# QData/FastSK

Measured on AMD Instinct MI355X. Metric: gkm kernel build: mismatch-combos/s, higher is better.
Workload: dtype u4 count planes (v_dot8_u32_u4), u32 register sums, u64 triangle (plain stores on the first pass over reset rows, else atomics); 1 GPU; config5: synthetic DNA 100000 x 300 bp, g=12 m=8 exact, 495 combos; n_seq=100000, seq_len=300, g=12, m=8, combos=495, parallelism=single GPU

## Files before the change

### fastsk_amd/csrc/fsk_engine_dense_shift.hip

```cpp
#include "fsk_engine_internal.h"
#include "fsk_kernels_dense_shift.h"

#include <map>

using namespace fsk_detail;

namespace fsk {

#define FSK_DMA_SHIFT 1
#define FSK_DMA_KERNEL k_dense_tile_shift
#define FSK_DMA_COMPACT 0
#include "fsk_tile_kernel_dma.inc"
#undef FSK_DMA_KERNEL
#undef FSK_DMA_SHIFT

#define FSK_DMA_SHIFT 2
#define FSK_DMA_KERNEL k_dense_tile_shift_all
#include "fsk_tile_kernel_dma.inc"
#undef FSK_DMA_KERNEL
#undef FSK_DMA_COMPACT
#undef FSK_DMA_SHIFT

}

// ... 101 lines not shown
int dense_shift_edge_keys(fsk_engine* e, const uint8_t* chunk_pos, uint32_t panels_pad) {
    ShiftPlan& p = e->shift;
    const uint32_t n_steps = (uint32_t)(p.steps.size() / 2), np_seq = panels_pad * fsk::PANEL;
    std::vector<uint32_t> steps = p.steps;
    dense_shift_unpack_flags(steps, p.n_bases, e->tune.dense_shift_batch != 0);
    const std::vector<uint32_t> chain_tab = dense_shift_chain_table(steps, p.n_bases);
    FSK_HIP(e->d_shift_steps.reserve(p.steps.size() + p.group_steps.size() + chain_tab.size()));
    FSK_HIP(e->d_edge_keys.reserve((size_t)n_steps * np_seq));
    FSK_HIP(hipMemcpyAsync(e->d_shift_steps.p, steps.data(), steps.size() * sizeof(uint32_t), hipMemcpyHostToDevice, e->stream));
    if (!p.group_steps.empty())
        FSK_HIP(hipMemcpyAsync(e->d_shift_steps.p + p.steps.size(), p.group_steps.data(), p.group_steps.size() * sizeof(uint32_t), hipMemcpyHostToDevice,
                               e->stream));
    if (!chain_tab.empty())
        FSK_HIP(hipMemcpyAsync(e->d_shift_steps.p + p.steps.size() + p.group_steps.size(), chain_tab.data(), chain_tab.size() * sizeof(uint32_t),
                               hipMemcpyHostToDevice, e->stream));
    e->ld.shift_chains = (uint32_t)(chain_tab.size() / 2);
    FSK_LAUNCH(fsk::k_dense_edge_keys, dim3(panels_pad, (n_steps + 3u) / 4u), dim3(256), 0, e->stream, e->view(), e->cfg.g, e->k, e->sigma, chunk_pos,
               (const uint32_t*)e->d_shift_steps.p, n_steps, np_seq, e->d_edge_keys.p);
    FSK_HIP(hipStreamSynchronize(e->stream));
    e->st.launches += 1;
    return FSK_OK;
}

int dense_shift_keymajor(fsk_engine* e, uint32_t panels_pad, int nb, uint32_t Vq8) {
    const ShiftPlan& p = e->shift;
    e->ld.shift_packed = false;
    if (e->tune.dense_shift_packed < 0 || p.max_chain != SHIFT_PACKED_CHAIN) return FSK_OK;
    const size_t plane = (size_t)panels_pad * Vq8 * fsk::PANEL * (size_t)nb;
    const size_t n_keys = (p.steps.size() / 2) * (size_t)panels_pad * fsk::PANEL;
    const size_t want = (2 * plane + n_keys) * sizeof(uint32_t);
    const char* why = nullptr;
    if (e->tune.dense_shift_plane_kb > 0 && want > (size_t)e->tune.dense_shift_plane_kb * 1024) why = "over the dense_shift_plane_kb cap";
    const size_t grow = (std::max(plane, e->d_KM.cap) - e->d_KM.cap + std::max(plane, e->d_KMH.cap) - e->d_KMH.cap +
                         std::max(n_keys, e->d_edge_offs.cap) - e->d_edge_offs.cap) * sizeof(uint32_t);
    if (!why && grow > 0) {
        size_t free_b = 0, total_b = 0;
        if (hipMemGetInfo(&free_b, &total_b) != hipSuccess) free_b = 0;
        if (grow > free_b / 2) why = "more than half of the free device memory";
        else if (e->d_KM.reserve(plane) != hipSuccess || e->d_KMH.reserve(plane) != hipSuccess || e->d_edge_offs.reserve(n_keys) != hipSuccess) {
            (void)hipGetLastError();
            e->d_KM.release(); e->d_KMH.release(); e->d_edge_offs.release();
            why = "hipMalloc failed";
        }
    }
    if (why) {
        if (e->trace())
            fprintf(stderr, "[fsk] dense shift classes: the key-major planes (%.1f MB) do not fit, %s: k_dense_shift_fix runs the corrections\n",
                    (double)want / 1e6, why);
        return FSK_OK;
    }
    const uint32_t n_pairs = panels_pad / 2u;
    const uint32_t kgrid = (uint32_t)(((size_t)n_pairs * nb * Vq8 * 16u + 255u) / 256u);
    FSK_LAUNCH(fsk::k_dense_keymajor, dim3(kgrid), dim3(256), 0, e->stream, (const uint32_t*)e->d_C4.p, n_pairs, nb, Vq8, e->d_KM.p);
    FSK_LAUNCH(fsk::k_dense_keymajor, dim3(kgrid), dim3(256), 0, e->stream, (const uint32_t*)e->d_C4H.p, n_pairs, nb, Vq8, e->d_KMH.p);
    FSK_LAUNCH(fsk::k_dense_edge_offs, dim3((uint32_t)((n_keys + 255u) / 256u)), dim3(256), 0, e->stream, (const uint16_t*)e->d_edge_keys.p, n_keys,
               e->d_edge_offs.p);
    e->st.launches += 3;
    e->ld.shift_packed = true;
    return FSK_OK;
}

int dense_shift_tiles(fsk_engine* e, u64 n_tiles, int nb, uint32_t Vq8, uint32_t nst, u64* K, int store, uint32_t panels_pad) {
    const ShiftPlan& p = e->shift;
    const bool one_launch = !p.group_steps.empty() && (e->tune.dense_shift_one_launch > 0 ||
                                                       (e->tune.dense_shift_one_launch == 0 && e->tune.tile_splits == 0 && n_tiles >= 16384));
    int base_launches = 1;
    if (one_launch) {
        FSK_LAUNCH(fsk::k_dense_tile_shift_all, dim3((uint32_t)n_tiles, 1), dim3(256), 0, e->stream, (const uint32_t*)e->d_C4.p,
                   (const uint32_t*)e->d_C4H.p, (const uint32_t*)e->d_rowmask.p, (const uint32_t*)e->d_tiletab.p, nb, Vq8, nst, (uint32_t)e->N, K,
                   (int)p.n_bases, store, (const uint32_t*)e->d_shift_steps.p + p.steps.size());
    } else {
        base_launches = (int)(p.groups.size() / 2);
        int slot0 = 0;
        for (size_t gi = 0; gi + 1 < p.groups.size(); gi += 2) {
            const int end = (int)p.groups[gi];
            FSK_LAUNCH(fsk::k_dense_tile_shift, dim3((uint32_t)n_tiles, 1), dim3(256), 0, e->stream, (const uint32_t*)e->d_C4.p,
                       (const uint32_t*)e->d_C4H.p, (const uint32_t*)e->d_rowmask.p, (const uint32_t*)e->d_tiletab.p, nb, Vq8, nst, (uint32_t)e->N, K,
                       end - slot0, gi == 0 ? store : 0, slot0, p.groups[gi + 1]);
            slot0 = end;
        }
    }
    if (e->ld.shift_packed) {
        const bool ahead = e->tune.dense_shift_inplace != 0 && e->tune.dense_shift_ahead != 0 && e->ld.shift_chains > 0;
        const auto k_packed = ahead ? fsk::k_dense_shift_packed<true, true>
                                    : e->tune.dense_shift_inplace != 0 ? fsk::k_dense_shift_packed<true, false> : fsk::k_dense_shift_packed<false, false>;
        FSK_LAUNCH(k_packed, dim3((uint32_t)n_tiles), dim3(256), 0, e->stream, (const uint32_t*)e->d_KM.p, (const uint32_t*)e->d_KMH.p,
                   (const uint32_t*)e->d_rowmask.p, (const uint32_t*)e->d_tiletab.p,
                   (const uint32_t*)e->d_shift_steps.p + (ahead ? p.steps.size() + p.group_steps.size() : 0), (uint32_t)(p.steps.size() / 2),
                   (const uint32_t*)e->d_edge_offs.p, panels_pad * fsk::PANEL, nb, Vq8, ahead ? e->ld.shift_chains : p.n_bases, (uint32_t)(30u * p.wsum), (uint32_t)e->N, K);
    } else {
        FSK_LAUNCH(fsk::k_dense_shift_fix, dim3((uint32_t)n_tiles), dim3(512), 0, e->stream, (const uint32_t*)e->d_C4.p, (const uint32_t*)e->d_C4H.p,
                   (const uint32_t*)e->d_rowmask.p, (const uint32_t*)e->d_tiletab.p, (const uint32_t*)e->d_shift_steps.p, (uint32_t)(p.steps.size() / 2),
                   (const uint16_t*)e->d_edge_keys.p, panels_pad * fsk::PANEL, nb, Vq8, (uint32_t)e->N, K);
    }
    e->st.launches += (int32_t)base_launches;
    return FSK_OK;
}

}
```

### fastsk_amd/csrc/fsk_engine_internal.h

```cpp
#pragma once
#include "fsk_common.h"

#include <algorithm>
#include <chrono>
#include <cmath>
#include <cstdarg>
#include <cstdio>
#include <cstdlib>
#include <cstring>
#include <string>
#include <array>
#include <atomic>
#include <thread>
#include <vector>

#include <cstdint>
#include <climits>

#include "../../include/fastsk_amd.h"
#include <condition_variable>
#include <functional>
#include <memory>
#include <mutex>

// ... 21 lines not shown
        hipError_t r = hipMalloc((void**)&p, n * sizeof(T));
        if (r == hipSuccess) cap = n;
        return r;
    }
    void release() {
        if (p) (void)hipFree(p);
        p = nullptr;
        cap = 0;
    }
};

template <typename T>
struct PinnedBuf {
    T* p = nullptr;
    size_t cap = 0;
    PinnedBuf() = default;
    PinnedBuf(PinnedBuf&& o) noexcept : p(o.p), cap(o.cap) { o.p = nullptr; o.cap = 0; }
    PinnedBuf& operator=(PinnedBuf&& o) noexcept { std::swap(p, o.p); std::swap(cap, o.cap); return *this; }
    ~PinnedBuf() { release(); }
    hipError_t reserve(size_t n, size_t slack = 0) {
        if (n <= cap) return hipSuccess;
        release();
        hipError_t r = hipHostMalloc((void**)&p, (n + slack) * sizeof(T));
        if (r == hipSuccess) cap = n + slack;
        return r;
    }
    void release() {
        if (p) (void)hipHostFree(p);
        p = nullptr;
        cap = 0;
    }
};

template <typename H, hipError_t (*Create)(H*, unsigned), hipError_t (*Destroy)(H)>
struct Handle {
    H h = nullptr;
    Handle() = default;
    Handle(Handle&& o) noexcept : h(o.h) { o.h = nullptr; }
    Handle& operator=(Handle&& o) noexcept { std::swap(h, o.h); return *this; }
    ~Handle() { if (h) (void)Destroy(h); }
    hipError_t create(unsigned flags) { return h ? hipSuccess : Create(&h, flags); }
    operator H() const { return h; }
};
using Stream = Handle<hipStream_t, hipStreamCreateWithFlags, hipStreamDestroy>;
using Event = Handle<hipEvent_t, hipEventCreateWithFlags, hipEventDestroy>;

struct DeviceScope {
    int prev = -1, dev;
    hipError_t err = hipSuccess;
    explicit DeviceScope(int d) : dev(d) {
        if (hipGetDevice(&prev) != hipSuccess) prev = -1;
        if (prev != dev) err = hipSetDevice(dev);
    }
    ~DeviceScope() {
        if (prev >= 0 && prev != dev) (void)hipSetDevice(prev);
    }
    DeviceScope(const DeviceScope&) = delete;
    DeviceScope& operator=(const DeviceScope&) = delete;
};
#define FSK_ON_DEVICE(e)                                                                      \
    DeviceScope fsk_on_device_((e)->cfg.device);                                             \
    if (fsk_on_device_.err != hipSuccess)                                                    \
        return (e)->fail(FSK_EDEVICE, "hipSetDevice(%d) failed: %s", (e)->cfg.device, hipGetErrorString(fsk_on_device_.err))

}

using fsk_detail::DevBuf;
using fsk_detail::PinnedBuf;
using fsk_detail::Stream;
using fsk_detail::Event;

#define FSK_TUNING_KEYS(X)                                                                                                          \
    X(trace, 0, 0, 1, "stderr: the tuning in force, where the host time of a load and of a variance-mode call goes")                 \
    X(profile, -1, -1, 2, "fsk_config.profile from here on (-1: as the engine was created)")                                          \
    X(compact, -1, -1, 1, "dense: key compaction off / on whatever the alphabet says (-1: a rare symbol decides)")                   \
    X(compact_rare, -1, -1, 1, "dense: keys that occur from the places of the rare symbols (1) or a marking pass over every window (0)") \
    X(tile_splits, 0, 0, 4096, "dense: combo splits per tile (0: by the size of the launch)")                                        \
    X(dense_small, 0, 0, 1, "dense: 1 = a split tile launch (small N) leaves its sums as 32-bit staging blocks that k_dense_widen adds into K (0: one 64-bit atomic a cell and split — measured faster: the atomics drain under other workgroups' dot products)")                                        \
    X(dense_shift, 0, -1, 1, "dense: one weighted Gram product per chain of shifted combinations, the other members by edge lookups (fsk_engine_dense_shift.hip) — 1 = whenever the call is eligible, -1 = never (0: when eligible, tile_splits = 0 and the launch has 16384 tiles or more, the size from which a tile has one workgroup anyway)") \
    X(dense_shift_packed, 0, -1, 0, "dense, shift classes: the derived steps from key-major planes, eight cells an LDS read (k_dense_keymajor, k_dense_shift_packed; chains cut at nine members) — 0 = whenever the shift path runs and the planes fit, -1 = never: k_dense_shift_fix on the count panels") \
    X(dense_shift_inplace, 1, 0, 1, "dense, shift classes: k_dense_shift_packed stages a chain's first planes and makes every further step's in LDS, one nibble up and one down a sequence (a step that meets a count above 15 in its tile, and the step behind it, are staged) — 0 = every step staged") \
    X(dense_shift_batch, 1, 0, 1, "dense, shift classes: k_dense_shift_packed adds the prefix sums of several steps byte to byte and hands the bytes to its int32 sums once a batch, where the step table says so (a step at chain position r counts 30 (r + 1) against a byte's 255; a batch may span chains) — 0 = after every step") \
    X(dense_shift_ahead, 1, 0, 1, "dense, shift classes: k_dense_shift_packed stages the NEXT chain's first planes and key offsets at a chain's first step, into the idle stage buffer and an offsets ring in LDS (80 KB a workgroup), and issues no vector memory load inside a chain (a chain that meets a count above 15 in its tile stages as before) — 0 = every chain start staged one step ahead; ignored with dense_shift_inplace = 0 and on the k_dense_shift_fix path") \
    X(dense_shift_one_launch, 0, -1, 1, "dense, shift classes: every chain-length group of the base products in ONE launch that flushes at the group ends without clearing (k_dense_tile_shift_all) — 1 = whenever the shift path runs, -1 = never: one k_dense_tile_shift launch a group (0: where the shift path runs by its own default rule, tile_splits = 0 and 16384 tiles or more)") \
    X(dense_shift_plane_kb, 0, 0, (int64_t)1 << 40, "dense, shift classes: the key-major planes and offsets may take this many KiB at most (0: half of the free memory; tests: the planes do not fit)") \
    X(dense_chunk, 0, 0, 1 << 24, "dense: cap of the count kernel's staging chunk, in windows (0: none)")                             \
    X(variance_dense_slots, 1, 0, 1, "variance mode, dense: 0 = zero fill + k_welford per iteration instead of storing slot triangles") \
    X(var_slots16, 1, 0, 1, "variance mode, sparse: 0 = u32 slot triangles from the start")                                          \
    X(sparse_global, 0, 0, 1, "sparse: every += as a 64-bit atomicAdd (k_sx_emit<DIRECT>) whatever N is")                             \
    X(sparse_unpacked, 0, 0, 1, "sparse: entries in the general 8 + 4 (+ 4) byte format whatever N is")                               \
    X(sparse_pairs, 1, 0, 1, "sparse: 0 = every update word 32 bits wide (1: unit products of clean runs travel two to a word)")      \
    X(sparse_sync, 0, 0, 1, "sparse: wait for every batch's word count and size its stream exactly")                                 \
    X(sparse_hint, 1, 0, 1, "sparse: 0 = the words per record of the previous set of sequences are never kept as a hint")             \
    X(sparse_exact_lanes, 0, 0, 2, "sparse: the batches of an exact accumulate never (1) / always (2) in two lanes (0: from six batches on)") \
    X(sparse_batch_records, 0, 0, (int64_t)1 << 31, "sparse: records per batch at most (0: 2^27)")                                   \
    X(guard_cap, 0, 0, (int64_t)1 << 40, "sparse: pretend the stream buffer holds this many words (0: its real size)")                \
    X(list_max_words, 0, 0, (int64_t)1 << 31, "sparse: update words of one batch beyond which its pairs go to K with atomics (0: 2^31)") \
    X(seg_scan_chunked, 0, 0, 1, "sparse: the three-launch segment scan whatever the tile count")                                    \
    X(extract_slots, 0, 0, 4, "sparse: slots per k_sx_extract_win workgroup, 1 or 4 (0: by the size of the launch)")                  \
    X(sparse_form, 0, 0, 3, "sparse: the update stage — 1 = owner bands whenever they exist, 2 = two-level blocks, 3 = 64-bit atomics (0: bands up to four LDS rounds a band, blocks beyond)") \
    X(blocks_sub_shift, 14, 4, 14, "sparse, blocks: log2 of the cells one k_sxb_consume workgroup sums in LDS (tests: small blocks on small inputs)") \
    X(blocks_max_bands, 512, 2, 512, "sparse, blocks: bands of one pass at most (tests: several passes on small inputs)")            \
    X(blocks_band_shift_max, 23, 4, 23, "sparse, blocks: log2 of a band's cells at most (tests)")                                    \
    X(blocks_pass_words, 0, 0, (int64_t)1 << 32, "sparse, blocks: update words of one pass at most (0: 2^31)")                       \
    X(sparse_desc, 0, -1, 1, "sparse, owner bands and two-level blocks: entries of many partners leave k_sx_emit as descriptors (one an entry; blocks: one per sub-band its partners fall into) that k_sx_consume / k_sxb_consume expand in LDS — 1 = always, -1 = never (0: once a batch of these sequences has shown sparse_desc_from pairs per record)") \
    X(sparse_desc_blocks, 1, 0, 1, "sparse, two-level blocks: 0 = never descriptors there (1: as sparse_desc says — one record per sub-band an entry's partners fall into)") \
    X(sparse_desc_cols, 1, 0, 3, "sparse, descriptors: where the partners are read from — 0 = the entries themselves; 1 = a column array (sequence id | multiplicity, 4 bytes) beside 8-byte entries, the entries themselves when they are packed (measured: 2-byte columns beside packed entries are no faster, 0.88 against 0.84 s in the large-g regime; 4-byte columns beside 8-byte entries 4.69 -> 4.44 ms a combo at N = 100k); tests: 2 = 4-byte columns always, 3 = 2-byte columns when N < 32768") \
    X(sparse_desc_min, 16, 1, 48, "sparse, descriptors: entries of more partners than this become descriptors (48: everything k_sx_emit does not bin in LDS; measured, large-g regime: 48 0.92 s, 32 0.85, 16 0.83-0.85, 8 0.88, 4 0.90)") \
    X(sparse_desc_from, 12, 1, 1 << 20, "sparse, descriptors: the pairs per sort record of a batch from which on the following batches use them (sparse_desc = 0)") \
    X(sparse_parts_target, 0, 0, 1 << 30, "sparse, owner bands: words of one k_sx_consume part (0: four LDS rounds' worth at least, 1/1024 of the batch's words; tests: several parts a band on small inputs)") \
    X(sparse_desc_parts, 2048, 1, 1 << 16, "sparse, descriptors: parts (k_sx_consume workgroups) the bands' streams are cut into, about") \
    X(sparse_share, 0, -1, 254, "sparse: leading kept positions sorted once per group of consecutive combos that share them (0: by cost; -1: never); batches of more than 16 slots only (smaller ones read their positions by id), and never when the presort's scratch passes a quarter of the free memory") \
    X(seed_splitmix, 0, 0, 1, "approx modes: 1 = fsk_set_seed draws the engine's older splitmix64 Fisher-Yates order (0: the reference's std::shuffle of minstd_rand0)") \
    X(mismatch_order, 0, 0, 1, "mismatch-weighted mode: 1 = the levels run from m = d down to 0 (0: from 0 up to d)")                   \
    X(collective, 0, 0, 2, "fsk_create_multi: FSK_COLL_* when fsk_config.collective is FSK_COLL_AUTO")                                \
    X(deadline_ms, 120000, -1, 86400000, "fsk_create_multi: the fail-fast bound when fsk_config.deadline_ms is 0 (negative: none)")   \
    X(svm_wg_max, 8192, 0, 8192, "fsk_svm_train: up to this many training rows the solver is one workgroup with alpha, G and y in LDS (k_svm_wg); beyond, two launches an iteration (k_svm_select_i / k_svm_select_j); 0 = always those") \
    X(svm_chunk, 256, 1, 65536, "fsk_svm_train: iterations enqueued between two reads of the solver's status record (k_svm_wg: iterations a launch)") \
    X(rows_tile, FSK_ROWS_TILE, FSK_ROWS_TILE, FSK_ROWS_TILE, "fsk_rows_build, read-only: the edge T of k_rows_syrk's tile of the rows kernel (compiled in)") \
    X(rows_panel, FSK_ROWS_PANEL, FSK_ROWS_PANEL, FSK_ROWS_PANEL, "fsk_rows_build, read-only: the consecutive train columns P a panel of k_rows_syrk stages in LDS (compiled in)") \
    FSK_TUNING_TEST_KEYS(X)
#ifdef FSK_TEST_HOOKS
#define FSK_TUNING_TEST_KEYS(X)                                            \
    X(fault_kind, 0, 0, 3, "test hook: 1 = host sleep, 2 = device spin before a band's collective; 3 = host sleep after the variance chains")   \
    X(fault_rank, -1, -1, 15, "test hook: the engine that is late")        \
    X(fault_band, -1, -1, 63, "test hook: before this band's collective")  \
    X(fault_ms, 0, 0, 60000, "test hook: by this many milliseconds")
#else
#define FSK_TUNING_TEST_KEYS(X)
#endif
struct fsk_tuning {
#define FSK_X(name, def, lo, hi, doc) int64_t name = (def);
    FSK_TUNING_KEYS(FSK_X)
#undef FSK_X
};

struct SxScratch {
    DevBuf<unsigned char> d_keys[2];
    DevBuf<uint32_t> d_blockhist, d_totals, d_tile_ent, d_ebase, d_Pk, d_Tk, d_ucount, d_uchunk, d_utot, d_list_off, d_ulist, d_part_base;
    DevBuf<u64> d_tile_stat;
    DevBuf<uint32_t> d_segc;
    DevBuf<int> d_tile_lrh, d_tile_rs, d_tile_lth, d_tile_ts;
    DevBuf<uint2> d_E;
    DevBuf<u64> d_sxstat;
    DevBuf<uint32_t> d_group_of, d_group_head, d_winp;
    DevBuf<unsigned char> d_part;
    DevBuf<uint32_t> d_ulist2, d_subcnt, d_suboff, d_subcur;
    DevBuf<uint32_t> d_dsubcnt, d_dsuboff, d_dsubcur;
    DevBuf<uint32_t> d_cols;
};

struct ShiftPlan {
    std::vector<int32_t> combos;
    u64 by_overflow = 0;
    std::vector<int32_t> order;
    std::vector<uint32_t> groups, steps, group_steps;
    uint32_t n_bases = 0;
    uint32_t max_chain = 0;
    u64 wsum = 0;
};

struct SvmCvState {
    bool valid = false;
    std::vector<double> oof;
    std::vector<fsk_svm_cv_score> scores;
    std::vector<fsk_svm_cv_problem> problems;
// ... 378 lines not shown
```

### fastsk_amd/csrc/fsk_kernels_dense_shift.h

```cpp
#pragma once
#include "fsk_bytesel.h"
#include "fsk_common.h"

namespace fsk {

__device__ __forceinline__ uint32_t panel_seq(uint32_t p) { return (p >> 2) + 16u * (p & 3u); }

__global__ __launch_bounds__(256) void k_dense_edge_keys(SeqView S, int g, int k, uint32_t sigma, const uint8_t* combo_pos, const uint32_t* steps,
                                                         uint32_t n_steps, uint32_t np_seq, uint16_t* keys) {
    const uint32_t r = threadIdx.x & 63u, step = blockIdx.y * 4u + (threadIdx.x >> 6), panel = blockIdx.x;
    if (step >= n_steps) return;
    const uint32_t seq = panel * PANEL + r;
    const uint32_t sl = steps[2u * step], up = sl >> 16, lo = sl & 0xffffu;
    uint32_t kd = 0, ks = 0;
    if (seq < S.n_seq) {
        const uint32_t len = S.len[seq], wbase = S.wstart[seq];
        if (len >= (uint32_t)g) {
            const uint32_t last = len - (uint32_t)g;
            for (int c = 0; c < k; ++c) {
                kd = kd * sigma + fetch_sym(S.words, wbase, (uint32_t)combo_pos[(size_t)lo * k + c], S.bits);
                ks = ks * sigma + fetch_sym(S.words, wbase, last + (uint32_t)combo_pos[(size_t)up * k + c], S.bits);
            }
        }
    }
// ... 79 lines not shown
            for (int q = 0; q < QW; ++q) {
                const uint32_t kk = (fsk_hw::readlane(kB, lsel + (uint32_t)q) >> hsh) & 0xffffu;
                edge(pb, (size_t)HALF, kk, mul, accR[0][q], accR[1][q]);
                if ((q & 3) == 3) asm volatile("" ::: "memory");
            }
#pragma unroll
            for (int q = 0; q < QW; ++q) {
                const uint32_t kk = (fsk_hw::readlane(kA, lsel + (uint32_t)q) >> hsh) & 0xffffu;
                edge(pb + 2 * HALF, (size_t)HALF, kk, mul, accC[0][q], accC[1][q]);
                if ((q & 3) == 3) asm volatile("" ::: "memory");
            }
        };
        lookups(wt);
        if (fl != 0u) {
            __syncthreads();
            load_stage(C4H, buf, sl);
            fsk_hw::wait_panel_rows();
            __syncthreads();
            lookups(16 * wt);
        }
        fsk_hw::wait_panel_rows();
        __syncthreads();
        sl_cur = sl_nxt; wt_cur = wt_nxt;
        sl_nxt = sl_n2; wt_nxt = wt_n2;
        buf ^= 1;
    }
    int* const T = reinterpret_cast<int*>(P);
#pragma unroll
    for (int h = 0; h < 2; ++h)
#pragma unroll
        for (int q = 0; q < QW; ++q) {
            const uint32_t i = (uint32_t)h * PANEL + lane, j = w * (uint32_t)QW + (uint32_t)q;
            T[i * TILE + ((j + i) & (TILE - 1u))] = accR[h][q];
        }
    __syncthreads();
#pragma unroll
    for (int h = 0; h < 2; ++h) {
        const uint32_t jd = (uint32_t)h * PANEL + lane;
        const u64 j = (u64)tj * TILE + (uint32_t)h * PANEL + panel_seq(lane);
#pragma unroll
        for (int q = 0; q < QW; ++q) {
            const uint32_t id = w * (uint32_t)QW + (uint32_t)q;
            const u64 i = (u64)ti * TILE + (id >> 6) * PANEL + panel_seq(id & 63u);
            const int v = accC[h][q] + T[id * TILE + ((jd + id) & (TILE - 1u))];
            if (i < N && j <= i && v != 0) atomicAdd(&K[tri_index(i, j)], (u64)(long long)v);
        }
    }
}

__device__ __forceinline__ uint32_t km_swizzle(uint32_t key) { return ((key >> 1) & 3u) << 2; }
__device__ __forceinline__ uint32_t km_offset(uint32_t key) { return key << 6 | km_swizzle(key) << 2; }

__global__ __launch_bounds__(256) void k_dense_keymajor(const uint32_t* plane, uint32_t n_pairs, int n_slots, uint32_t Vq8, uint32_t* KM) {
    const size_t id = (size_t)blockIdx.x * 256u + threadIdx.x;
    const uint32_t t = (uint32_t)id & 15u;
    size_t rest = id >> 4;
    const uint32_t row = (uint32_t)(rest % Vq8);
    rest /= Vq8;
    const uint32_t slot = (uint32_t)(rest % (uint32_t)n_slots);
    const size_t pair = rest / (uint32_t)n_slots;
    if (pair >= n_pairs) return;
    const size_t slot_stride = (size_t)Vq8 * PANEL, panel_stride = (size_t)n_slots * slot_stride;
    const uint32_t* src = plane + 2u * pair * panel_stride + slot * slot_stride + (size_t)row * PANEL + 4u * t;
    const uint4 a = *reinterpret_cast<const uint4*>(src), b = *reinterpret_cast<const uint4*>(src + panel_stride);
    const uint32_t in[8] = {a.x, a.y, a.z, a.w, b.x, b.y, b.z, b.w};
    uint32_t* out = KM + (pair * (size_t)n_slots + slot) * ((size_t)Vq8 * 128u);
#pragma unroll
    for (uint32_t q = 0; q < 8u; ++q) {
        uint32_t v = 0;
#pragma unroll
        for (uint32_t n = 0; n < 8u; ++n) v |= ((in[n] >> (4u * q)) & 15u) << (4u * n);
        const uint32_t key = row * 8u + q;
        out[key * 16u + (t ^ km_swizzle(key))] = v;
    }
}

__global__ __launch_bounds__(256) void k_dense_edge_offs(const uint16_t* keys, size_t n, uint32_t* offs) {
    const size_t q = (size_t)blockIdx.x * 256u + threadIdx.x;
    if (q >= n) return;
    const uint32_t kk = keys[q];
    offs[q] = km_offset(kk & 255u) | km_offset(kk >> 8) << 16;
}

template <bool INPLACE, bool AHEAD = false>
__global__ __launch_bounds__(256, 2) void k_dense_shift_packed(const uint32_t* KM, const uint32_t* KMH, const uint32_t* rowmask, const uint32_t* tile_tab,
                                                               const uint32_t* steps, uint32_t n_steps, const uint32_t* offs, uint32_t np_seq,
                                                               int n_slots, uint32_t Vq8, uint32_t n_bases, uint32_t bias, uint32_t N, u64* K) {
    static_assert(INPLACE || !AHEAD, "the ahead schedule is a schedule of the in-place form");
    constexpr uint32_t SIDE = 256u * 16u;
    constexpr uint32_t PBUF = 2u * SIDE;
    constexpr uint32_t RING = 8u * 256u;
    __shared__ __attribute__((aligned(1024))) uint32_t P[AHEAD ? 2 * PBUF + 2 * RING : 2 * PBUF];
    const uint32_t tid = threadIdx.x, lane = tid & 63u;
    const uint32_t w = (uint32_t)__builtin_amdgcn_readfirstlane(tid >> 6);
    const uint32_t M4 = (uint32_t)__builtin_amdgcn_readfirstlane(fsk_hw::vgpr_copy(0x0f0f0f0fu));
    const uint32_t tr = (w >> 1) * 8u + (lane >> 3), tc = (w & 1u) * 8u + (lane & 7u);
    const uint32_t tile = tile_tab[blockIdx.x];
    const uint32_t ti = tile >> 16, tj = tile & 0xffffu;
    const size_t slot_stride = (size_t)Vq8 * 128u;
    const size_t pair_stride = (size_t)n_slots * slot_stride;
    const uint32_t side_bytes = Vq8 * 512u;

    uint32_t acc[8][8], Rr[2][8], Rc[2][8], Qr[2][8], Qc[2][8];
#pragma unroll
    for (int a = 0; a < 8; ++a) {
#pragma unroll
        for (int b = 0; b < 8; ++b) acc[a][b] = 0u;
        Rr[0][a] = Rr[1][a] = Rc[0][a] = Rc[1][a] = 0u;
        Qr[0][a] = Qr[1][a] = Qc[0][a] = Qc[1][a] = 0u;
    }

    const fsk_hw::lds_addr_t lds_wave = fsk_hw::lds_address(P) + w * 1024u;
    auto load_stage = [&](const uint32_t* plane, uint32_t buf, uint32_t sl) {
        const uint32_t up = sl >> 16, lo = sl & 0xffffu;
#pragma unroll
        for (uint32_t side = 0; side < 2u; ++side) {
            const uint32_t* src = plane + (side == 0u ? ti : tj) * pair_stride + (size_t)(side == 0u ? up : lo) * slot_stride;
#pragma unroll
            for (uint32_t q = 0; q < 4u; ++q)
                if (q * 4096u < side_bytes)
                    fsk_hw::panel_rows_to_lds(src, side_bytes, lds_wave + (buf * PBUF + side * SIDE + q * 1024u) * 4u, q * 4096u + tid * 16u);
        }
    };
    auto load_offs = [&](uint32_t s, uint4 (&oR)[2], uint4 (&oC)[2]) {
        const uint32_t* os = offs + (size_t)s * np_seq;
#pragma unroll
        for (uint32_t h = 0; h < 2u; ++h) {
            oR[h] = *reinterpret_cast<const uint4*>(os + ti * TILE + h * PANEL + 4u * tr);
            oC[h] = *reinterpret_cast<const uint4*>(os + tj * TILE + h * PANEL + 4u * tc);
        }
    };
    auto flagged = [&](uint32_t sl) {
        const uint32_t up = sl >> 16, lo = sl & 0xffffu;
        const uint32_t mA = rowmask[(size_t)(ti * 2u) * n_slots + up] | rowmask[(size_t)(ti * 2u + 1u) * n_slots + up];
        const uint32_t mB = rowmask[(size_t)(tj * 2u) * n_slots + lo] | rowmask[(size_t)(tj * 2u + 1u) * n_slots + lo];
        return mA | mB;
    };
    auto lds_at = [&](uint32_t byte_off) { return *reinterpret_cast<const uint32_t*>(reinterpret_cast<const char*>(P) + byte_off); };

    uint32_t sl, wt, fl, sn = 0u, wn = 0u;
    uint32_t s2 = 0u, w2 = 0u, fl_nx = 0u;
    uint4 oR_n[2], oC_n[2];
    uint32_t buf = 0;
    [[maybe_unused]] uint32_t* const ring = P + 2u * PBUF;
    [[maybe_unused]] uint32_t cb = 0u, dv0 = 0u, dv1 = 0u;
    [[maybe_unused]] uint32_t c = 0u, r = 0u, rem = 0u;
    [[maybe_unused]] uint32_t n0 = 0u, n1 = 0u, mk_n = 0u;
    [[maybe_unused]] uint32_t flw = 0u, wu = 0u, slq = 0u;
    [[maybe_unused]] uint32_t half = 0u, rg = 0u;
    [[maybe_unused]] bool lost = false;
    [[maybe_unused]] auto enter_chain = [&](uint32_t e0, uint32_t e1, uint32_t mk) {
        flw = (uint32_t)__ballot(fsk_hw::vgpr_copy(mk) != 0u);
        sl = e0;
        slq = ((e0 >> 16) + 1u) << 16 | (e0 >> 16);
        rem = e1 & 15u;
        wt = (e1 >> 8) & 255u;
        wu = e1 >> 16;
        r = 0u;
        rg = half * RING;
    };
    [[maybe_unused]] auto load_desc = [&]() {
        const uint32_t q = cb + lane < n_bases ? cb + lane : n_bases - 1u;
        dv0 = steps[2u * q];
        dv1 = steps[2u * q + 1u];
    };
    [[maybe_unused]] auto load_masks = [&](uint32_t e0, uint32_t e1) {
        const uint32_t mr = lane >> 2, x = lane & 3u, up0 = e0 >> 16;
        uint32_t m = 0u;
        if (mr < (e1 & 15u)) {
            const uint32_t slot = x < 2u ? up0 + mr : (mr == 0u ? (e0 & 0xffffu) : up0 + mr - 1u);
            m = rowmask[(size_t)((x < 2u ? ti : tj) * 2u + (x & 1u)) * n_slots + slot];
        }
        return m;
    };
    [[maybe_unused]] auto load_ring = [&](uint32_t hf, uint32_t s_first, uint32_t n) {
        const uint32_t ring_lane = lane < 32u ? (ti * TILE + 4u * lane) * 4u : (tj * TILE + 4u * (lane - 32u)) * 4u;
#pragma unroll
        for (uint32_t q = 0; q < 2u; ++q) {
            const uint32_t rr = w + 4u * q;
            if (rr < n)
                fsk_hw::panel_rows_to_lds(offs + (size_t)(s_first + rr) * np_seq, np_seq * 4u, fsk_hw::lds_address(ring) + (hf * RING + rr * 256u) * 4u,
                                          ring_lane);
        }
    };
    [[maybe_unused]] auto ring_offs = [&](uint32_t at, uint4 (&oR)[2], uint4 (&oC)[2]) {
        const uint32_t* q = ring + at;
#pragma unroll
        for (uint32_t hh = 0; hh < 2u; ++hh) {
            oR[hh] = *reinterpret_cast<const uint4*>(q + hh * PANEL + 4u * tr);
            oC[hh] = *reinterpret_cast<const uint4*>(q + TILE + hh * PANEL + 4u * tc);
        }
    };
    if constexpr (AHEAD) {
        load_desc();
        const uint32_t d0 = fsk_hw::readlane(dv0, 0u), d1 = fsk_hw::readlane(dv1, 0u);
        const uint32_t mk = load_masks(d0, d1);
        load_stage(KM, 0u, d0);
        load_ring(0u, 0u, d1 & 15u);
        fsk_hw::wait_panel_rows();
        __syncthreads();
        fl = 0u;
        enter_chain(d0, d1, mk);
        ring_offs(0u, oR_n, oC_n);
    } else {
        sl = steps[0]; wt = steps[1]; fl = flagged(sl);
        sn = n_steps > 1u ? steps[2] : 0u; wn = n_steps > 1u ? steps[3] : 0u;
        if constexpr (INPLACE) {
            if (n_steps > 2u) { s2 = steps[4]; w2 = steps[5]; }
            if (n_steps > 1u) fl_nx = flagged(sn);
        }
        load_offs(0u, oR_n, oC_n);
        load_stage(KM, 0u, sl);
        fsk_hw::wait_panel_rows();
        __syncthreads();
    }
    for (uint32_t s = 0; s < n_steps; ++s) {
        uint32_t oR[8], oC[8];
#pragma unroll
        for (int h = 0; h < 2; ++h) {
            oR[4 * h] = fsk_hw::vgpr_copy(oR_n[h].x); oR[4 * h + 1] = fsk_hw::vgpr_copy(oR_n[h].y);
            oR[4 * h + 2] = fsk_hw::vgpr_copy(oR_n[h].z); oR[4 * h + 3] = fsk_hw::vgpr_copy(oR_n[h].w);
            oC[4 * h] = fsk_hw::vgpr_copy(oC_n[h].x); oC[4 * h + 1] = fsk_hw::vgpr_copy(oC_n[h].y);
            oC[4 * h + 2] = fsk_hw::vgpr_copy(oC_n[h].z); oC[4 * h + 3] = fsk_hw::vgpr_copy(oC_n[h].w);
        }
        bool same;
        uint32_t uo_n = 0u;
        [[maybe_unused]] bool last = false;
        if constexpr (AHEAD) {
            const bool first = r == 0u, has_next = c + 1u < n_bases;
            last = rem == 1u;
            if (first) {
                lost = false;
                if (has_next) {
                    if (c + 1u - cb >= 64u) {
                        cb = c;
                        load_desc();
                    }
                    n0 = fsk_hw::readlane(dv0, c + 1u - cb);
                    n1 = fsk_hw::readlane(dv1, c + 1u - cb);
                    mk_n = load_masks(n0, n1);
                }
            }
            fl = flw & 15u;
            wt = (wt & 255u) | (wu & 1u) << 8;
            same = !last && (flw & 255u) == 0u;
            if (first && has_next) {
                if (last || same) load_stage(KM, buf ^ 1u, n0);
                else lost = true;
                load_ring(half ^ 1u, s + rem, n1 & 15u);
            }
            if (!last) {
                ring_offs(rg + 256u, oR_n, oC_n);
                if (same) {
                    uo_n = ring[rg + (w < 2u ? 256u : (uint32_t)TILE) + (tid & 127u)];
                } else {
                    lost = true;
                    if (!first) fsk_hw::wait_panel_rows();
                    load_stage(KM, buf ^ 1u, slq);
                }
            } else if (lost && has_next) {
                load_stage(KM, buf ^ 1u, n0);
            }
        } else {
            same = INPLACE && s + 1u < n_steps && (sn & 0xffffu) >= n_bases && fl == 0u && fl_nx == 0u;
            if (s + 1u < n_steps) {
                load_offs(s + 1u, oR_n, oC_n);
                if (same) uo_n = offs[(size_t)(w < 2u ? s + 1u : s) * np_seq + (w < 2u ? ti : tj) * TILE + (tid & 127u)];
                else load_stage(KM, buf ^ 1u, sn);
            }
        }
        if (AHEAD ? r == 0u : (sl & 0xffffu) < n_bases) {
#pragma unroll
            for (int a = 0; a < 8; ++a) Rr[0][a] = Rr[1][a] = Rc[0][a] = Rc[1][a] = 0u;
        }
        const uint32_t baseA = buf * PBUF * 4u, baseB = baseA + SIDE * 4u;
        const uint32_t xA = (tr * 4u) | baseA, xB = (tc * 4u) | baseB;
        uint32_t dA[8], sA[8], dB[8], sB[8];
        auto read_A = [&](int e) { dA[e] = lds_at(fsk_hw::xor_word<0>(oC[e], xA)); sA[e] = lds_at(fsk_hw::xor_word<1>(oC[e], xA)); };
        auto read_B = [&](int e) { dB[e] = lds_at(fsk_hw::xor_word<0>(oR[e], xB)); sB[e] = lds_at(fsk_hw::xor_word<1>(oR[e], xB)); };
        auto row_term = [&](int e) {
            Rr[0][e] += (sA[e] & M4) + (~dA[e] & M4);
            Rr[1][e] += ((sA[e] >> 4) & M4) + (~(dA[e] >> 4) & M4);
            Qr[0][e] += Rr[0][e];
            Qr[1][e] += Rr[1][e];
        };
        auto col_term = [&](int e) {
            Rc[0][e] += (sB[e] & M4) + (~dB[e] & M4);
            Rc[1][e] += ((sB[e] >> 4) & M4) + (~(dB[e] >> 4) & M4);
            Qc[0][e] += Rc[0][e];
            Qc[1][e] += Rc[1][e];
        };
#pragma unroll
        for (int e = 0; e < 8; ++e) read_A(e);
        fsk_hw::first_use(dA[0], sA[0], dA[1], sA[1], dA[2], sA[2], dA[3], sA[3]);
#pragma unroll
        for (int e = 0; e < 4; ++e) read_B(e);
#pragma unroll
        for (int e = 0; e < 4; ++e) row_term(e);
        fsk_hw::first_use(dA[4], sA[4], dA[5], sA[5], dA[6], sA[6], dA[7], sA[7]);
// ... 130 lines not shown
```

Measured before the change: 472.1 combos/s.

## Run chains without high counts as a straight loop in the ahead schedule

Adds a STRAIGHT variant of k_dense_shift_packed, on by default, that handles each chain as a tight inner loop. Each step does its lookups, then a barrier, the in-place LDS update and a barrier, with the step counter, ring position and unpack bits carried in registers. Chains that meet a count above 15 keep a fallback path inside the same loop. The aim is to drop the per-step branching and bookkeeping of the general step loop, at the cost of a much larger kernel body and more register pressure.

```diff
diff --git a/fastsk_amd/csrc/fsk_engine_dense_shift.hip b/fastsk_amd/csrc/fsk_engine_dense_shift.hip
--- a/fastsk_amd/csrc/fsk_engine_dense_shift.hip
+++ b/fastsk_amd/csrc/fsk_engine_dense_shift.hip
@@ -207,8 +207,13 @@
     }
     if (e->ld.shift_packed) {
         const bool ahead = e->tune.dense_shift_inplace != 0 && e->tune.dense_shift_ahead != 0 && e->ld.shift_chains > 0;
-        const auto k_packed = ahead ? fsk::k_dense_shift_packed<true, true>
-                                    : e->tune.dense_shift_inplace != 0 ? fsk::k_dense_shift_packed<true, false> : fsk::k_dense_shift_packed<false, false>;
+        const bool straight = ahead && e->tune.dense_shift_straight != 0;
+        const auto k_packed = straight ? fsk::k_dense_shift_packed<true, true, true>
+                              : ahead  ? fsk::k_dense_shift_packed<true, true, false>
+                                       : e->tune.dense_shift_inplace != 0 ? fsk::k_dense_shift_packed<true, false, false> : fsk::k_dense_shift_packed<false, false, false>;
+        if (e->trace())
+            fprintf(stderr, "[fsk] dense shift classes: the corrections by k_dense_shift_packed<%s>\n",
+                    straight ? "true, true, true" : ahead ? "true, true, false" : e->tune.dense_shift_inplace != 0 ? "true, false, false" : "false, false, false");
         FSK_LAUNCH(k_packed, dim3((uint32_t)n_tiles), dim3(256), 0, e->stream, (const uint32_t*)e->d_KM.p, (const uint32_t*)e->d_KMH.p,
                    (const uint32_t*)e->d_rowmask.p, (const uint32_t*)e->d_tiletab.p,
                    (const uint32_t*)e->d_shift_steps.p + (ahead ? p.steps.size() + p.group_steps.size() : 0), (uint32_t)(p.steps.size() / 2),
diff --git a/fastsk_amd/csrc/fsk_engine_internal.h b/fastsk_amd/csrc/fsk_engine_internal.h
--- a/fastsk_amd/csrc/fsk_engine_internal.h
+++ b/fastsk_amd/csrc/fsk_engine_internal.h
@@ -127,6 +127,7 @@
     X(dense_shift_inplace, 1, 0, 1, "dense, shift classes: k_dense_shift_packed stages a chain's first planes and makes every further step's in LDS, one nibble up and one down a sequence (a step that meets a count above 15 in its tile, and the step behind it, are staged) — 0 = every step staged") \
     X(dense_shift_batch, 1, 0, 1, "dense, shift classes: k_dense_shift_packed adds the prefix sums of several steps byte to byte and hands the bytes to its int32 sums once a batch, where the step table says so (a step at chain position r counts 30 (r + 1) against a byte's 255; a batch may span chains) — 0 = after every step") \
     X(dense_shift_ahead, 1, 0, 1, "dense, shift classes: k_dense_shift_packed stages the NEXT chain's first planes and key offsets at a chain's first step, into the idle stage buffer and an offsets ring in LDS (80 KB a workgroup), and issues no vector memory load inside a chain (a chain that meets a count above 15 in its tile stages as before) — 0 = every chain start staged one step ahead; ignored with dense_shift_inplace = 0 and on the k_dense_shift_fix path") \
+    X(dense_shift_straight, 1, 0, 1, "dense, shift classes: the ahead schedule of k_dense_shift_packed runs a chain none of whose steps meets a count above 15 in its tile as a straight loop (lookups; barrier, update, barrier) that carries a step counter, the ring position and the unpack bits, and every other chain by the step loop of dense_shift_ahead — 0 = every chain by that step loop; ignored wherever dense_shift_ahead is ignored") \
     X(dense_shift_one_launch, 0, -1, 1, "dense, shift classes: every chain-length group of the base products in ONE launch that flushes at the group ends without clearing (k_dense_tile_shift_all) — 1 = whenever the shift path runs, -1 = never: one k_dense_tile_shift launch a group (0: where the shift path runs by its own default rule, tile_splits = 0 and 16384 tiles or more)") \
     X(dense_shift_plane_kb, 0, 0, (int64_t)1 << 40, "dense, shift classes: the key-major planes and offsets may take this many KiB at most (0: half of the free memory; tests: the planes do not fit)") \
     X(dense_chunk, 0, 0, 1 << 24, "dense: cap of the count kernel's staging chunk, in windows (0: none)")                             \
diff --git a/fastsk_amd/csrc/fsk_kernels_dense_shift.h b/fastsk_amd/csrc/fsk_kernels_dense_shift.h
--- a/fastsk_amd/csrc/fsk_kernels_dense_shift.h
+++ b/fastsk_amd/csrc/fsk_kernels_dense_shift.h
@@ -185,11 +185,12 @@
     offs[q] = km_offset(kk & 255u) | km_offset(kk >> 8) << 16;
 }
 
-template <bool INPLACE, bool AHEAD = false>
+template <bool INPLACE, bool AHEAD = false, bool STRAIGHT = false>
 __global__ __launch_bounds__(256, 2) void k_dense_shift_packed(const uint32_t* KM, const uint32_t* KMH, const uint32_t* rowmask, const uint32_t* tile_tab,
                                                                const uint32_t* steps, uint32_t n_steps, const uint32_t* offs, uint32_t np_seq,
                                                                int n_slots, uint32_t Vq8, uint32_t n_bases, uint32_t bias, uint32_t N, u64* K) {
     static_assert(INPLACE || !AHEAD, "the ahead schedule is a schedule of the in-place form");
+    static_assert(AHEAD || !STRAIGHT, "the straight chains are a form of the ahead schedule's loop");
     constexpr uint32_t SIDE = 256u * 16u;
     constexpr uint32_t PBUF = 2u * SIDE;
     constexpr uint32_t RING = 8u * 256u;
@@ -317,7 +318,177 @@
         fsk_hw::wait_panel_rows();
         __syncthreads();
     }
-    for (uint32_t s = 0; s < n_steps; ++s) {
+    if constexpr (STRAIGHT) {
+        uint32_t s = 0u;
+        uint32_t xA = tr * 4u, xB = (tc * 4u) | (SIDE * 4u);
+        uint32_t oR[8], oC[8], dA[8], sA[8], dB[8], sB[8];
+        auto read_A = [&](int e) { dA[e] = lds_at(fsk_hw::xor_word<0>(oC[e], xA)); sA[e] = lds_at(fsk_hw::xor_word<1>(oC[e], xA)); };
+        auto read_B = [&](int e) { dB[e] = lds_at(fsk_hw::xor_word<0>(oR[e], xB)); sB[e] = lds_at(fsk_hw::xor_word<1>(oR[e], xB)); };
+        auto row_term = [&](int e) {
+            Rr[0][e] += (sA[e] & M4) + (~dA[e] & M4);
+            Rr[1][e] += ((sA[e] >> 4) & M4) + (~(dA[e] >> 4) & M4);
+            Qr[0][e] += Rr[0][e];
+            Qr[1][e] += Rr[1][e];
+        };
+        auto col_term = [&](int e) {
+            Rc[0][e] += (sB[e] & M4) + (~dB[e] & M4);
+            Rc[1][e] += ((sB[e] >> 4) & M4) + (~(dB[e] >> 4) & M4);
+            Qc[0][e] += Rc[0][e];
+            Qc[1][e] += Rc[1][e];
+        };
+        const uint32_t mk_r = lane >> 2, mk_x = lane & 3u;
+        const size_t mk_row = (size_t)((mk_x < 2u ? ti : tj) * 2u + (mk_x & 1u)) * n_slots;
+        const uint32_t mk_add = mk_r - (mk_x >> 1), mk_base = fsk_hw::vgpr_copy(mk_x >= 2u && mk_r == 0u ? 1u : 0u);
+        auto next_masks = [&](uint32_t e0, uint32_t e1) {
+            const uint32_t up0 = e0 >> 16, slot = up0 + mk_add + mk_base * ((e0 & 0xffffu) + 1u - up0);
+            uint32_t m = 0u;
+            if (mk_r < (e1 & 15u)) m = rowmask[mk_row + slot];
+            return m;
+        };
+        auto next_offs = [&](uint32_t at) {
+            const uint32_t* q = ring + at;
+#pragma unroll
+            for (uint32_t hh = 0; hh < 2u; ++hh) {
+                const uint4 a = *reinterpret_cast<const uint4*>(q + hh * PANEL + 4u * tr), b = *reinterpret_cast<const uint4*>(q + TILE + hh * PANEL + 4u * tc);
+                oR[4 * hh] = a.x; oR[4 * hh + 1] = a.y; oR[4 * hh + 2] = a.z; oR[4 * hh + 3] = a.w;
+                oC[4 * hh] = b.x; oC[4 * hh + 1] = b.y; oC[4 * hh + 2] = b.z; oC[4 * hh + 3] = b.w;
+            }
+        };
+#pragma unroll
+        for (int h = 0; h < 2; ++h) {
+            oR[4 * h] = oR_n[h].x; oR[4 * h + 1] = oR_n[h].y; oR[4 * h + 2] = oR_n[h].z; oR[4 * h + 3] = oR_n[h].w;
+            oC[4 * h] = oC_n[h].x; oC[4 * h + 1] = oC_n[h].y; oC[4 * h + 2] = oC_n[h].z; oC[4 * h + 3] = oC_n[h].w;
+        }
+        while (c < n_bases) {
+            const uint32_t gen = flw;
+            lost = false;
+            if (c + 1u < n_bases) {
+                if (c + 1u - cb >= 64u) {
+                    cb = c;
+                    load_desc();
+                }
+                n0 = fsk_hw::readlane(dv0, c + 1u - cb);
+                n1 = fsk_hw::readlane(dv1, c + 1u - cb);
+                mk_n = next_masks(n0, n1);
+                s += rem;
+                if (rem == 1u || (flw & 255u) == 0u) load_stage(KM, buf ^ 1u, n0);
+                else lost = true;
+                load_ring(half ^ 1u, s, n1 & 15u);
+            }
+#pragma unroll
+            for (int a = 0; a < 8; ++a) Rr[0][a] = Rr[1][a] = Rc[0][a] = Rc[1][a] = 0u;
+            for (;;) {
+                const bool last = rem == 1u;
+                bool in_place = true;
+                uint32_t uo_n = 0u;
+                bool hi = false;
+                if (gen == 0u) {
+                    if (!last) uo_n = ring[rg + (w < 2u ? 256u : (uint32_t)TILE) + (tid & 127u)];
+                } else {
+                    hi = (flw & 15u) != 0u;
+                    in_place = (flw & 255u) == 0u;
+                    if (!last) {
+                        if (in_place) {
+                            uo_n = ring[rg + (w < 2u ? 256u : (uint32_t)TILE) + (tid & 127u)];
+                        } else {
+                            lost = true;
+                            fsk_hw::wait_panel_rows();
+                            load_stage(KM, buf ^ 1u, ((sl >> 16) + 1u) << 16 | (sl >> 16));
+                        }
+                    } else if (lost && c + 1u < n_bases) {
+                        load_stage(KM, buf ^ 1u, n0);
+                    }
+                }
+#pragma unroll
+                for (int e = 0; e < 8; ++e) read_A(e);
+                fsk_hw::first_use(dA[0], sA[0], dA[1], sA[1], dA[2], sA[2], dA[3], sA[3]);
+#pragma unroll
+                for (int e = 0; e < 4; ++e) read_B(e);
+#pragma unroll
+                for (int e = 0; e < 4; ++e) row_term(e);
+                fsk_hw::first_use(dA[4], sA[4], dA[5], sA[5], dA[6], sA[6], dA[7], sA[7]);
+#pragma unroll
+                for (int e = 4; e < 8; ++e) read_B(e);
+                if (!last && !hi) next_offs(rg + 256u);
+#pragma unroll
+                for (int e = 4; e < 8; ++e) row_term(e);
+                fsk_hw::first_use(dB[0], sB[0], dB[1], sB[1], dB[2], sB[2], dB[3], sB[3]);
+#pragma unroll
+                for (int e = 0; e < 4; ++e) col_term(e);
+                fsk_hw::first_use(dB[4], sB[4], dB[5], sB[5], dB[6], sB[6], dB[7], sB[7]);
+#pragma unroll
+                for (int e = 4; e < 8; ++e) col_term(e);
+                if ((wu & 1u) != 0u) {
+#pragma unroll
+                    for (int e = 0; e < 8; ++e) {
+                        acc[0][e] = fsk_hw::add_byte<0>(acc[0][e], Qr[0][e]); acc[1][e] = fsk_hw::add_byte<0>(acc[1][e], Qr[1][e]);
+                        acc[2][e] = fsk_hw::add_byte<1>(acc[2][e], Qr[0][e]); acc[3][e] = fsk_hw::add_byte<1>(acc[3][e], Qr[1][e]);
+                        acc[4][e] = fsk_hw::add_byte<2>(acc[4][e], Qr[0][e]); acc[5][e] = fsk_hw::add_byte<2>(acc[5][e], Qr[1][e]);
+                        acc[6][e] = fsk_hw::add_byte<3>(acc[6][e], Qr[0][e]); acc[7][e] = fsk_hw::add_byte<3>(acc[7][e], Qr[1][e]);
+                    }
+#pragma unroll
+                    for (int e = 0; e < 8; ++e) {
+                        acc[e][0] = fsk_hw::add_byte<0>(acc[e][0], Qc[0][e]); acc[e][1] = fsk_hw::add_byte<0>(acc[e][1], Qc[1][e]);
+                        acc[e][2] = fsk_hw::add_byte<1>(acc[e][2], Qc[0][e]); acc[e][3] = fsk_hw::add_byte<1>(acc[e][3], Qc[1][e]);
+                        acc[e][4] = fsk_hw::add_byte<2>(acc[e][4], Qc[0][e]); acc[e][5] = fsk_hw::add_byte<2>(acc[e][5], Qc[1][e]);
+                        acc[e][6] = fsk_hw::add_byte<3>(acc[e][6], Qc[0][e]); acc[e][7] = fsk_hw::add_byte<3>(acc[e][7], Qc[1][e]);
+                        Qr[0][e] = Qr[1][e] = Qc[0][e] = Qc[1][e] = 0u;
+                    }
+                }
+                if (hi) {
+                    __syncthreads();
+                    load_stage(KMH, buf, sl);
+                    fsk_hw::wait_panel_rows();
+                    __syncthreads();
+                    const uint32_t mul = 16u * wt;
+#pragma unroll
+                    for (int e = 0; e < 8; ++e) {
+                        read_A(e);
+                        read_B(e);
+#pragma unroll
+                        for (int n = 0; n < 8; ++n) {
+                            acc[n][e] += (((sA[e] >> (4 * n)) & 15u) - ((dA[e] >> (4 * n)) & 15u)) * mul;
+                            acc[e][n] += (((sB[e] >> (4 * n)) & 15u) - ((dB[e] >> (4 * n)) & 15u)) * mul;
+                        }
+                    }
+                    if (!last) next_offs(rg + 256u);
+                }
+                if (last) break;
+                if (in_place) {
+                    fsk_hw::barrier_lds_only();
+                    const uint32_t uo = fsk_hw::vgpr_copy(uo_n), od = uo & 0xffffu, os = uo >> 16;
+                    if (od != os) {
+                        const uint32_t p = tid & 127u, t4 = p & 0x3cu, e = (p >> 6) * 4u + (p & 3u);
+                        const uint32_t base = buf * PBUF + (w >> 1) * SIDE, inc = 1u << (4u * e);
+                        atomicAdd(&P[base + ((os ^ t4) >> 2)], inc);
+                        atomicAdd(&P[base + ((od ^ t4) >> 2)], 0u - inc);
+                    }
+                    fsk_hw::barrier_lds_only();
+                } else {
+                    fsk_hw::wait_panel_rows();
+                    __syncthreads();
+                    buf ^= 1u;
+                    xA ^= PBUF * 4u; xB ^= PBUF * 4u;
+                }
+                if (gen != 0u) {
+                    sl = ((sl >> 16) + 1u) << 16 | (sl >> 16);
+                    --wt; flw >>= 4;
+                }
+                --rem; wu >>= 1; rg += 256u;
+            }
+            fsk_hw::wait_panel_rows();
+            __syncthreads();
+            buf ^= 1u;
+            xA ^= PBUF * 4u; xB ^= PBUF * 4u;
+            if (c + 1u < n_bases) {
+                half ^= 1u;
+                enter_chain(n0, n1, mk_n);
+                next_offs(rg);
+            }
+            ++c;
+        }
+    }
+    for (uint32_t s = 0; !STRAIGHT && s < n_steps; ++s) {
         uint32_t oR[8], oC[8];
 #pragma unroll
         for (int h = 0; h < 2; ++h) {
```

After: 479.4 combos/s (median of 6 runs). +1.6%, better.
